# Inspector-Butters/light-client-consensus-specs

Measured on AMD Instinct MI355X. Metric: verified LightClientUpdates/sec (512-member committee), higher is better.
Workload: dtype u32 (381-bit Montgomery Fp on 12x32-bit limbs; SHA-256 words)

## Files before the change

### light-client-consensus-specs_amd/csrc/lcv_curve.hpp

```cpp
#pragma once
#include "lcv_tower.hpp"

namespace lcv {

LCV_FN void f_add(fp& r, const fp& a, const fp& b) { fp_add(r, a, b); }
LCV_FN void f_add(fp2& r, const fp2& a, const fp2& b) { fp2_add(r, a, b); }
LCV_FN void f_sub(fp& r, const fp& a, const fp& b) { fp_sub(r, a, b); }
LCV_FN void f_sub(fp2& r, const fp2& a, const fp2& b) { fp2_sub(r, a, b); }
LCV_FN void f_dbl(fp& r, const fp& a) { fp_dbl(r, a); }
LCV_FN void f_dbl(fp2& r, const fp2& a) { fp2_dbl(r, a); }
LCV_FN void f_neg(fp& r, const fp& a) { fp_neg(r, a); }
LCV_FN void f_neg(fp2& r, const fp2& a) { fp2_neg(r, a); }
LCV_FN void f_mul(fp& r, const fp& a, const fp& b) { fp_mul(r, a, b); }
LCV_FN void f_mul(fp2& r, const fp2& a, const fp2& b) { fp2_mul(r, a, b); }
LCV_FN void f_sqr(fp& r, const fp& a) { fp_sqr(r, a); }
LCV_FN void f_sqr(fp2& r, const fp2& a) { fp2_sqr(r, a); }
LCV_FN void f_inv(fp& r, const fp& a) { fp_inv(r, a); }
LCV_FN void f_inv(fp2& r, const fp2& a) { fp2_inv(r, a); }
LCV_FN bool f_is_zero(const fp& a) { return fp_is_zero(a); }
LCV_FN bool f_is_zero(const fp2& a) { return fp2_is_zero(a); }
LCV_FN bool f_eq(const fp& a, const fp& b) { return fp_eq(a, b); }
LCV_FN bool f_eq(const fp2& a, const fp2& b) { return fp2_eq(a, b); }
LCV_FN void f_one(fp& r) { fp_one(r); }
LCV_FN void f_one(fp2& r) { fp2_one(r); }
// ... 195 lines not shown
  if (xz) return aflag ? PT_BAD : PT_INF;
  if (!fp_raw_lt_p(xr)) return PT_BAD;
  fp x, g, y, chk, four;
  fp_to_mont(x, xr);
  fp_sqr(g, x);
  fp_mul(g, g, x);
  LCV_FP_SET(four, LCV_FOUR_INIT);
  fp_add(g, g, four);
  fp_pow_p1d4(y, g);
  fp_sqr(chk, y);
  if (!fp_eq(chk, g)) return PT_BAD;
  if (fp_is_large(y) != (aflag != 0)) fp_neg(y, y);
  r.x = x;
  r.y = y;
  return PT_OK;
}

LCV_FN void g1_compress(uint8_t* out, const g1a& p, bool inf) {
  if (inf) {
    out[0] = 0xc0;
    for (int i = 1; i < 48; ++i) out[i] = 0;
    return;
  }
  fp_to_be48(out, p.x);
  out[0] |= 0x80 | (fp_is_large(p.y) ? 0x20 : 0);
}

LCV_FN bool g1_in_subgroup(const g1a& p) {
  g1j t, u;
  jac_from_aff(t, p);
  LCV_NOUNROLL for (int i = 62; i >= 0; --i) {
    jac_dbl(t, t);
    if ((LCV_X_ABS >> i) & 1ull) jac_madd(t, t, p);
  }
  u = t;
  LCV_NOUNROLL for (int i = 62; i >= 0; --i) {
    jac_dbl(u, u);
    if ((LCV_X_ABS >> i) & 1ull) jac_add(u, u, t);
  }
  if (jac_is_inf(u)) return false;
  fp z2, z3, beta, a, b, ny;
  fp_sqr(z2, u.z);
  fp_mul(z3, z2, u.z);
  LCV_FP_SET(beta, LCV_G1_BETA_INIT);
  fp_mul(a, beta, p.x);
  fp_mul(a, a, z2);
  fp_neg(ny, p.y);
  fp_mul(b, ny, z3);
  return fp_eq(a, u.x) && fp_eq(b, u.y);
}

LCV_FN void g2_generator(g2a& r) { LCV_FP2_SET(r.x, LCV_G2X); LCV_FP2_SET(r.y, LCV_G2Y); }

LCV_FN int g2_decompress(g2a& r, const uint8_t* in) {
  const uint32_t b0 = in[0];
  const uint32_t cflag = (b0 >> 7) & 1u, bflag = (b0 >> 6) & 1u, aflag = (b0 >> 5) & 1u;
  fp x1r, x0r;
  fp_raw_from_be48(x1r, in);
  x1r.v[11] &= 0x1fffffffu;
  fp_raw_from_be48(x0r, in + 48);
  const uint32_t xz = (fp_is_zero(x1r) && fp_is_zero(x0r)) ? 1u : 0u;
  if (!cflag || bflag != xz) return PT_BAD;
  if (xz) return aflag ? PT_BAD : PT_INF;
  if (!fp_raw_lt_p(x1r) || !fp_raw_lt_p(x0r)) return PT_BAD;
  fp2 x, g, y, b;
  fp_to_mont(x.c0, x0r);
  fp_to_mont(x.c1, x1r);
  fp2_sqr(g, x);
  fp2_mul(g, g, x);
  LCV_FP2_SET(b, LCV_B2);
  fp2_add(g, g, b);
  if (!fp2_sqrt(y, g)) return PT_BAD;
  const bool large = fp_is_zero(y.c1) ? fp_is_large(y.c0) : fp_is_large(y.c1);
  if (large != (aflag != 0)) fp2_neg(y, y);
  r.x = x;
  r.y = y;
  return PT_OK;
}

LCV_FN void g2_compress(uint8_t* out, const g2a& p, bool inf) {
  if (inf) {
    out[0] = 0xc0;
    for (int i = 1; i < 96; ++i) out[i] = 0;
    return;
  }
  fp_to_be48(out, p.x.c1);
  fp_to_be48(out + 48, p.x.c0);
  const bool large = fp_is_zero(p.y.c1) ? fp_is_large(p.y.c0) : fp_is_large(p.y.c1);
  out[0] |= 0x80 | (large ? 0x20 : 0);
}

LCV_FN void g2_psi(g2j& r, const g2j& p) {
  fp2 cx, cy;
  LCV_FP2_SET(cx, LCV_PSI_CX);
  LCV_FP2_SET(cy, LCV_PSI_CY);
  fp2_conj(r.x, p.x);
  fp2_mul(r.x, r.x, cx);
  fp2_conj(r.y, p.y);
  fp2_mul(r.y, r.y, cy);
  fp2_conj(r.z, p.z);
}

LCV_FN bool g2_in_subgroup(const g2a& p) {
  g2j t;
  jac_mul_xabs_aff(t, p);
  if (jac_is_inf(t)) return false;
  fp2 cx, cy, px, py, z2, z3, a, b;
  LCV_FP2_SET(cx, LCV_PSI_CX);
  LCV_FP2_SET(cy, LCV_PSI_CY);
  fp2_conj(px, p.x);
  fp2_mul(px, px, cx);
  fp2_conj(py, p.y);
  fp2_mul(py, py, cy);
  fp2_sqr(z2, t.z);
  fp2_mul(z3, z2, t.z);
  fp2_mul(a, px, z2);
  fp2_mul(b, py, z3);
  fp2_neg(b, b);
  return fp2_eq(a, t.x) && fp2_eq(b, t.y);
}

LCV_FN void g2_clear_cofactor(g2j& r, const g2j& p) {
  g2j t1, t2, t3, u;
  jac_mul_x(t1, p);
  g2_psi(t2, p);
  jac_dbl(t3, p);
  g2_psi(t3, t3);
  g2_psi(t3, t3);
  jac_neg(u, t2);
  jac_add(t3, t3, u);
  jac_add(t2, t1, t2);
// ... 10 lines not shown
```

### light-client-consensus-specs_amd/csrc/lcv_field.hpp

```cpp
#pragma once
#include "lcv_common.hpp"
#include "lcv_consts.inc"
#include "lcv_col28.hpp"
#include "lcv_wave.hpp"

namespace lcv {

struct fp { uint32_t v[12]; };
struct fp2 { fp c0, c1; };

#define LCV_FP_SET(r, INIT) do { constexpr uint32_t _lcv_k[12] = INIT; LCV_UNROLL for (int _i = 0; _i < 12; ++_i) (r).v[_i] = _lcv_k[_i]; } while (0)
#define LCV_FP2_SET(r, NAME) do { LCV_FP_SET((r).c0, NAME##_C0); LCV_FP_SET((r).c1, NAME##_C1); } while (0)

LCV_FN void fp_zero(fp& r) { LCV_UNROLL for (int i = 0; i < 12; ++i) r.v[i] = 0; }
LCV_FN void fp_one(fp& r) { LCV_FP_SET(r, LCV_ONE_INIT); }
LCV_FN bool fp_is_zero(const fp& a) {
  uint32_t x = 0;
  LCV_UNROLL for (int i = 0; i < 12; ++i) x |= a.v[i];
  return x == 0;
}
LCV_FN bool fp_eq(const fp& a, const fp& b) {
  uint32_t x = 0;
  LCV_UNROLL for (int i = 0; i < 12; ++i) x |= a.v[i] ^ b.v[i];
  return x == 0;
// ... 172 lines not shown
#else
LCV_FN void fp_sqr(fp& r, const fp& a) { fp_mul(r, a, a); }
#endif

#define LCV_DEF_POW(fname, EXPARR, NBITS)                                  \
  LCV_FN void fname(fp& r, const fp& a) {                                  \
    fp acc = a;                                                            \
    LCV_NOUNROLL for (int i = (NBITS) - 2; i >= 0; --i) {                  \
      fp_sqr(acc, acc);                                                    \
      if ((EXPARR[i >> 5] >> (i & 31)) & 1u) fp_mul(acc, acc, a);          \
    }                                                                      \
    r = acc;                                                               \
  }
LCV_DEF_POW(fp_inv_fermat, LCV_EXP_P_MINUS_2, LCV_EXP_P_MINUS_2_BITS)
#define LCV_DEF_POW_W4(fname, EXPARR, NBITS)                                              \
  LCV_FN void fname(fp& r, const fp& a) {                                                 \
    fp tab[8], a2;                                                                        \
    tab[0] = a;                                                                           \
    fp_sqr(a2, a);                                                                        \
    LCV_UNROLL for (int k = 1; k < 8; ++k) fp_mul(tab[k], tab[k - 1], a2);               \
    fp acc = a;                                                                           \
    bool started = false;                                                                 \
    int i = (NBITS) - 1;                                                                  \
    LCV_NOUNROLL while (i >= 0) {                                                         \
      if (!((EXPARR[i >> 5] >> (i & 31)) & 1u)) {                                         \
        fp_sqr(acc, acc);                                                                 \
        --i;                                                                              \
        continue;                                                                         \
      }                                                                                   \
      int j = i - 3 < 0 ? 0 : i - 3;                                                      \
      while (!((EXPARR[j >> 5] >> (j & 31)) & 1u)) ++j;                                   \
      uint32_t w = 0;                                                                     \
      for (int k = i; k >= j; --k) {                                                      \
        w = (w << 1) | ((EXPARR[k >> 5] >> (k & 31)) & 1u);                               \
        if (started) fp_sqr(acc, acc);                                                    \
      }                                                                                   \
      fp m = tab[0];                                                                      \
      LCV_UNROLL for (int k = 1; k < 8; ++k) if ((w >> 1) == (uint32_t)k) m = tab[k];     \
      if (started) fp_mul(acc, acc, m); else acc = m;                                     \
      started = true;                                                                     \
      i = j - 1;                                                                          \
    }                                                                                     \
    r = acc;                                                                              \
  }
#ifndef LCV_POW_LF
#if defined(LCV_CPU_FAST)
#define LCV_POW_LF 0
#elif defined(LCV_HOSTSIM)
#define LCV_POW_LF 1
#else
#define LCV_POW_LF 2
#endif
#endif
#if LCV_POW_LF
LCV_FN void fp_lf_in(uint32_t L[14], const fp& a) {
  fp c, t;
  LCV_FP_SET(c, LCV_2E392_RAW_INIT);
  fp_mul(t, a, c);
  sop_to28<12, 14>(L, t.v);
}
LCV_FN void fp_lf_out(fp& r, const uint32_t L[14]) {
  uint32_t w[12];
  LCV_UNROLL for (int k = 0; k < 12; ++k) {
    const int b = 32 * k, j = b / 28, s = b % 28;
    uint32_t x = L[j] >> s;
    if (j + 1 < 14) x |= L[j + 1] << (28 - s);
    if (s > 24 && j + 2 < 14) x |= L[j + 2] << (56 - s);
    w[k] = x;
  }
  fp t, c;
  fp_reduce_once(t.v, w);
  LCV_FP_SET(c, LCV_2E376_RAW_INIT);
  fp_mul(r, t, c);
}
#define LCV_POW_WB (LCV_POW_LF == 2 ? 3 : 4)
#define LCV_POW_TAB(k, q) tabh[k][q]
#define LCV_POW_TAB_DECL uint32_t tabh[1 << (LCV_POW_WB - 1)][14];
#define LCV_POW_TAB_GET(m, idx)                                                           \
  LCV_UNROLL for (int q = 0; q < 14; ++q) m[q] = tabh[0][q];                              \
  LCV_UNROLL for (int k = 1; k < (1 << (LCV_POW_WB - 1)); ++k)                             \
    if ((idx) == (uint32_t)k) LCV_UNROLL for (int q = 0; q < 14; ++q) m[q] = tabh[k][q];
#define LCV_DEF_POW_LF(fname, EXPARR, NBITS)                                              \
  LCV_FN void fname(fp& r, const fp& a_) {                                                \
    uint32_t a[14], t[14], a2[14], acc[14];                                               \
    LCV_POW_TAB_DECL                                                                      \
    fp_lf_in(a, a_);                                                                      \
    LCV_UNROLL for (int j = 0; j < 14; ++j) LCV_POW_TAB(0, j) = a[j];                     \
    fp_sqr_lf(a2, a);                                                                     \
    LCV_UNROLL for (int j = 0; j < 14; ++j) t[j] = a[j];                                  \
    LCV_UNROLL for (int k = 1; k < (1 << (LCV_POW_WB - 1)); ++k) {                         \
      fp_mul_lf(t, t, a2);                                                                \
      LCV_UNROLL for (int j = 0; j < 14; ++j) LCV_POW_TAB(k, j) = t[j];                   \
    }                                                                                     \
    LCV_UNROLL for (int j = 0; j < 14; ++j) acc[j] = a[j];                                \
    bool started = false;                                                                 \
    int i = (NBITS) - 1;                                                                  \
    LCV_NOUNROLL while (i >= 0) {                                                         \
      if (!((EXPARR[i >> 5] >> (i & 31)) & 1u)) {                                         \
        fp_sqr_lf(acc, acc);                                                              \
        --i;                                                                              \
        continue;                                                                         \
      }                                                                                   \
      int j = i - (LCV_POW_WB - 1) < 0 ? 0 : i - (LCV_POW_WB - 1);                         \
      while (!((EXPARR[j >> 5] >> (j & 31)) & 1u)) ++j;                                   \
      uint32_t w = 0;                                                                     \
      for (int k = i; k >= j; --k) {                                                      \
        w = (w << 1) | ((EXPARR[k >> 5] >> (k & 31)) & 1u);                               \
        if (started) fp_sqr_lf(acc, acc);                                                 \
      }                                                                                   \
      uint32_t m[14];                                                                     \
      LCV_POW_TAB_GET(m, w >> 1)                                                          \
      if (started) fp_mul_lf(acc, acc, m);                                                \
      else LCV_UNROLL for (int q = 0; q < 14; ++q) acc[q] = m[q];                         \
      started = true;                                                                     \
      i = j - 1;                                                                          \
    }                                                                                     \
    fp_lf_out(r, acc);                                                                    \
  }
#if defined(__HIP_DEVICE_COMPILE__) && LCV_POW_LF == 3
#define LCV_DEF_POW_WAVE(fname, SCHED, NSCHED)                                            \
  LCV_FN void fname(fp& r, const fp& a_) {                                                \
    WaveTabs T;                                                                           \
    wv_tabs(T);                                                                           \
    uint32_t L[14];                                                                       \
    fp_lf_in(L, a_);                                                                      \
    const uint32_t a = wv_scatter(L);                                                     \
    uint32_t tab[8];                                                                      \
    tab[0] = a;                                                                           \
    const uint32_t a2 = wv_mul(a, a, T);                                                  \
    LCV_UNROLL for (int k = 1; k < 8; ++k) tab[k] = wv_mul(tab[k - 1], a2, T);            \
    uint32_t e = SCHED[0], acc = tab[0];                                                  \
    LCV_UNROLL for (int k = 1; k < 8; ++k) acc = (e >> 16) == (uint32_t)k ? tab[k] : acc; \
    LCV_NOUNROLL for (int t = 1; t < (NSCHED); ++t) {                                     \
      e = SCHED[t];                                                                       \
      LCV_NOUNROLL for (uint32_t q = e & 0xFFFFu; q > 0; --q) acc = wv_mul(acc, acc, T);  \
      const uint32_t idx = e >> 16;                                                       \
      if (idx != 0xFFFFu) {                                                               \
        uint32_t m = tab[0];                                                              \
        LCV_UNROLL for (int k = 1; k < 8; ++k) m = idx == (uint32_t)k ? tab[k] : m;        \
        acc = wv_mul(acc, m, T);                                                          \
      }                                                                                   \
    }                                                                                     \
    wv_gather(L, acc);                                                                    \
    fp_lf_out(r, L);                                                                      \
  }
// ... 157 lines not shown
    eta = by_divsteps30(eta, (uint32_t)f.v[0], (uint32_t)g.v[0], t);
    by_update_de(d, e, t);
    by_update_fg(f, g, t);
    int32_t z = 0;
    LCV_UNROLL for (int k = 0; k < 13; ++k) z |= g.v[k];
    if (z == 0) break;
  }
  uint32_t x[13];
  LCV_UNROLL for (int w = 0; w < 13; ++w) x[w] = 0;
  LCV_UNROLL for (int k = 0; k < 12; ++k) {
    const int b = 30 * k, w = b >> 5, s = b & 31;
    x[w] |= (uint32_t)d.v[k] << s;
    if (s > 2) x[w + 1] |= (uint32_t)d.v[k] >> (32 - s);
  }
  x[11] |= (uint32_t)d.v[12] << 8;
  x[12] = (uint32_t)(d.v[12] >> 24);
  LCV_UNROLL for (int pass = 0; pass < 2; ++pass) {
    const uint32_t m = 0u - (x[12] >> 31);
    uint32_t c = 0;
    LCV_UNROLL for (int j = 0; j < 12; ++j) x[j] = addc32(x[j], PL[j] & m, c, c);
    x[12] = x[12] + c;
  }
  uint32_t nz = 0;
  LCV_UNROLL for (int j = 0; j < 12; ++j) nz |= x[j];
  const uint32_t neg = (f.v[12] < 0 && nz != 0) ? 0xFFFFFFFFu : 0u;
  fp y;
  uint32_t br = 0;
  LCV_UNROLL for (int j = 0; j < 12; ++j) {
    const uint32_t n = subc32(PL[j], x[j], br, br);
    y.v[j] = neg ? n : x[j];
  }
  fp r3;
  LCV_FP_SET(r3, LCV_R3_INIT);
  fp_mul(r, y, r3);
}

LCV_FN void fp_inv(fp& r, const fp& a) { fp_inv_by(r, a); }

LCV_FN void fp2_zero(fp2& r) { fp_zero(r.c0); fp_zero(r.c1); }
LCV_FN void fp2_one(fp2& r) { fp_one(r.c0); fp_zero(r.c1); }
LCV_FN bool fp2_is_zero(const fp2& a) { return fp_is_zero(a.c0) && fp_is_zero(a.c1); }
LCV_FN bool fp2_eq(const fp2& a, const fp2& b) { return fp_eq(a.c0, b.c0) && fp_eq(a.c1, b.c1); }
LCV_FN void fp2_sel(fp2& r, bool c, const fp2& a, const fp2& b) { fp_sel(r.c0, c, a.c0, b.c0); fp_sel(r.c1, c, a.c1, b.c1); }
LCV_FN void fp2_add(fp2& r, const fp2& a, const fp2& b) { fp_add(r.c0, a.c0, b.c0); fp_add(r.c1, a.c1, b.c1); }
LCV_FN void fp2_sub(fp2& r, const fp2& a, const fp2& b) { fp_sub(r.c0, a.c0, b.c0); fp_sub(r.c1, a.c1, b.c1); }
LCV_FN void fp2_dbl(fp2& r, const fp2& a) { fp_dbl(r.c0, a.c0); fp_dbl(r.c1, a.c1); }
LCV_FN void fp2_neg(fp2& r, const fp2& a) { fp_neg(r.c0, a.c0); fp_neg(r.c1, a.c1); }
LCV_FN void fp2_half(fp2& r, const fp2& a) { fp_half(r.c0, a.c0); fp_half(r.c1, a.c1); }
LCV_FN void fp2_conj(fp2& r, const fp2& a) { r.c0 = a.c0; fp_neg(r.c1, a.c1); }
LCV_FN void fp2_mul_fp(fp2& r, const fp2& a, const fp& s) { fp_mul(r.c0, a.c0, s); fp_mul(r.c1, a.c1, s); }

LCV_FN void fp2_mul(fp2& r, const fp2& a, const fp2& b) {
  fp t0, t1, t2, t3;
  fp_mul(t0, a.c0, b.c0);
  fp_mul(t1, a.c1, b.c1);
  fp_add(t2, a.c0, a.c1);
  fp_add(t3, b.c0, b.c1);
  fp_mul(t2, t2, t3);
  fp_sub(r.c0, t0, t1);
  fp_sub(t2, t2, t0);
  fp_sub(r.c1, t2, t1);
}
LCV_FN void fp2_sqr(fp2& r, const fp2& a) {
  fp t0, t1, t2;
  fp_add(t0, a.c0, a.c1);
  fp_sub(t1, a.c0, a.c1);
  fp_mul(t2, a.c0, a.c1);
  fp_mul(r.c0, t0, t1);
  fp_dbl(r.c1, t2);
}
LCV_FN void fp2_mul_xi(fp2& r, const fp2& a) {
  fp t;
  fp_sub(t, a.c0, a.c1);
  fp_add(r.c1, a.c0, a.c1);
  r.c0 = t;
}
LCV_FN void fp2_inv(fp2& r, const fp2& a) {
  fp t0, t1;
  fp_sqr(t0, a.c0);
  fp_sqr(t1, a.c1);
  fp_add(t0, t0, t1);
  fp_inv(t1, t0);
  fp_mul(r.c0, a.c0, t1);
  fp_mul(t0, a.c1, t1);
  fp_neg(r.c1, t0);
}
LCV_FN void fp2_norm(fp& n, const fp2& a) {
  fp t;
  fp_sqr(n, a.c0);
  fp_sqr(t, a.c1);
  fp_add(n, n, t);
}

LCV_FN bool fp2_sqrt_alpha(fp2& y, const fp2& a, const fp& alpha) {
  const bool a1z = fp_is_zero(a.c1);
  fp delta;
  fp_add(delta, a.c0, alpha);
  fp_half(delta, delta);
  fp_sel(delta, a1z, a.c0, delta);
  fp t, c, s;
  fp_pow_p3d4(t, delta);
  fp_mul(c, t, delta);
  fp_mul(s, c, t);
  fp one;
  fp_one(one);
  const bool s_one = fp_eq(s, one);
  fp u, nu;
  fp_half(u, a.c1);
  fp_mul(u, u, t);
  fp_neg(nu, u);
  fp zero;
  fp_zero(zero);
  const bool first = a1z ? (s_one || fp_is_zero(delta)) : s_one;
  fp y0a, y1a;
  fp_sel(y0a, a1z, zero, nu);
  fp_sel(y1a, a1z, zero, u);
  fp_sel(y.c0, first, c, y0a);
  fp_sel(y.c1, first, y1a, c);
  fp2 chk;
  fp2_sqr(chk, y);
  return fp2_eq(chk, a);
}
LCV_FN bool fp2_sqrt(fp2& y, const fp2& a) {
  fp n, alpha;
  fp2_norm(n, a);
  fp_pow_p1d4(alpha, n);
  return fp2_sqrt_alpha(y, a, alpha);
}
LCV_FN bool fp2_is_square_alpha(const fp2& a, fp& alpha) {
  fp n, chk;
  fp2_norm(n, a);
  fp_pow_p1d4(alpha, n);
  fp_sqr(chk, alpha);
  return fp_eq(chk, n);
}
LCV_FN uint32_t fp2_sgn0(const fp2& a) {
  fp r0, r1;
  fp_from_mont(r0, a.c0);
  fp_from_mont(r1, a.c1);
  const uint32_t sign0 = r0.v[0] & 1u;
  const uint32_t zero0 = fp_is_zero(r0) ? 1u : 0u;
  const uint32_t sign1 = r1.v[0] & 1u;
  return sign0 | (zero0 & sign1);
}

}
```

### light-client-consensus-specs_amd/csrc/lcv_functors.hpp

```cpp
#pragma once
#include "lcv_items.hpp"

using namespace lcv;

struct F_nsc_team {
  BatchDev B; CommitteeDev C; Work W;
  static constexpr uint32_t TEAM = NSC_TEAM, LDS_WORDS = NSC_LDS, SHARED_WORDS = 0;
  LCV_HD uint32_t rounds() const { return NSC_ROUNDS; }
  LCV_HD void operator()(uint32_t j, uint32_t lane, uint32_t r, uint32_t* lds, uint32_t*) const { item_nsc_team(j, lane, r, lds, B, C, W); }
};
struct F_pre { BatchDev B; CommitteeDev C; Params P; Work W; LCV_HD void operator()(uint32_t i) const { item_pre(i, B, C, P, W); } };
struct F_sigroot { BatchDev B; Params P; Work W; LCV_HD void operator()(uint32_t i) const { item_sigroot(i, B, P, W); } };
struct F_h2c_map { Work W; LCV_HD void operator()(uint32_t t) const { item_h2c_map(t, W); } };
struct F_sig { BatchDev B; Work W; LCV_HD void operator()(uint32_t i) const { item_sig(i, B, W); } };
struct F_h2c_map_lat { Work W; LCV_HD void operator()(uint32_t t) const { item_h2c_map(t, W); } };
struct F_sig_lat { BatchDev B; Work W; LCV_HD void operator()(uint32_t i) const { item_sig(i, B, W); } };
struct F_agg { BatchDev B; CommitteeDev C; Work W; LCV_HD void operator()(uint32_t i) const { item_agg(i, B, C, W); } };
struct F_agg_fold { Work W; uint32_t m; LCV_HD void operator()(uint32_t) const { item_agg_fold(m, W); } };
struct F_verdict { Work W; LCV_HD void operator()(uint32_t i) const { item_verdict(i, W); } };
struct F_key { CommitteeDev C; LCV_HD void operator()(uint32_t t) const { item_committee_key(t, C); } };
struct F_agg_team {
  BatchDev B; CommitteeDev C; Work W;
  static constexpr uint32_t TEAM = AGG_TEAM, LDS_WORDS = AGG_LDS, SHARED_WORDS = 0;
  LCV_HD uint32_t rounds() const { return AGG_ROUNDS; }
  LCV_HD void operator()(uint32_t i, uint32_t lane, uint32_t r, uint32_t* lds, uint32_t*) const {
    item_agg_team(i, lane, r, lds, B, C, W);
  }
};
struct F_sum {
  CommitteeDev C;
  static constexpr uint32_t TEAM = SUM_TEAM, LDS_WORDS = SUM_LDS, SHARED_WORDS = 0;
  LCV_HD uint32_t rounds() const { return SUM_ROUNDS; }
  LCV_HD void operator()(uint32_t c, uint32_t lane, uint32_t r, uint32_t* lds, uint32_t*) const {
    item_committee_sum_team(c, lane, r, lds, C);
  }
};

struct F_msg_import {
  const uint8_t* msg; Work W;
  LCV_HD void operator()(uint32_t i) const {
    h256 m;
    LCV_UNROLL for (int k = 0; k < 8; ++k) m.w[k] = ld_be32(msg + 32 * (size_t)i + 4 * k);
    soa_st_h256(W.msg, W.cap, i, m);
  }
};
struct F_msg_import_b0 {
  const uint8_t* msg; uint64_t len; Work W;
  LCV_HD void operator()(uint32_t i) const {
    h256 b0;
    xmd_b0_bytes(b0, msg, len);
    soa_st_h256(W.msg, W.cap, i, b0);
  }
};
struct F_merkle {
  const uint8_t* leaf; const uint8_t* branch; const uint8_t* root; uint8_t* out; uint32_t depth; uint64_t index;
  LCV_HD void operator()(uint32_t i) const {
    h256 l, r;
    ld_chunk(l, leaf + 32 * (size_t)i);
    ld_chunk(r, root + 32 * (size_t)i);
    out[i] = merkle_branch_ok(l, branch + (size_t)32 * depth * i, (int)depth, index, r) ? 1 : 0;
  }
};
struct F_htr_sc {
  const uint8_t* sc; uint8_t* out;
  LCV_HD void operator()(uint32_t i) const {
    h256 r;
    htr_sync_committee(r, sc + (size_t)K_SC * i);
// ... 137 lines not shown
```

### light-client-consensus-specs_amd/csrc/lcv_h2c.hpp

```cpp
#pragma once
#include "lcv_curve.hpp"
#include "lcv_sha.hpp"

namespace lcv {

LCV_FN void xmd_next(h256& out, const h256& b0, const h256& prev, uint32_t i) {
  constexpr uint32_t C1T[8] = LCV_XMD_C1_TAIL_INIT;
  constexpr uint32_t C2[16] = LCV_XMD_C2_INIT;
  uint32_t st[8], blk[16];
  sha256_iv(st);
  LCV_UNROLL for (int k = 0; k < 8; ++k) { blk[k] = b0.w[k] ^ prev.w[k]; blk[8 + k] = C1T[k]; }
  blk[8] |= i << 24;
  sha256_compress(st, blk);
  LCV_UNROLL for (int k = 0; k < 16; ++k) blk[k] = C2[k];
  sha256_compress(st, blk);
  LCV_UNROLL for (int k = 0; k < 8; ++k) out.w[k] = st[k];
}

LCV_FN void xmd_b0(h256& b0, const h256& msg) {
  constexpr uint32_t H1[8] = LCV_XMD_H1_INIT;
  constexpr uint32_t B2T[8] = LCV_XMD_B2_TAIL_INIT;
  constexpr uint32_t B3[16] = LCV_XMD_B3_INIT;
  uint32_t st[8], blk[16];
  LCV_UNROLL for (int k = 0; k < 8; ++k) { st[k] = H1[k]; blk[k] = msg.w[k]; blk[8 + k] = B2T[k]; }
  sha256_compress(st, blk);
  LCV_UNROLL for (int k = 0; k < 16; ++k) blk[k] = B3[k];
  sha256_compress(st, blk);
  LCV_UNROLL for (int k = 0; k < 8; ++k) b0.w[k] = st[k];
}

LCV_FN void fp_from_xmd64(fp& r, const h256& hi, const h256& lo) {
  fp h, l, c, t;
  LCV_UNROLL for (int k = 0; k < 8; ++k) { h.v[k] = hi.w[7 - k]; l.v[k] = lo.w[7 - k]; }
  LCV_UNROLL for (int k = 8; k < 12; ++k) { h.v[k] = 0; l.v[k] = 0; }
  LCV_FP_SET(c, LCV_C256_INIT);
  fp_mul(t, h, c);
  LCV_FP_SET(c, LCV_R2_INIT);
  fp_mul(r, l, c);
  fp_add(r, r, t);
}

LCV_FN void iso_map_g2(g2j& r, const fp2& x, const fp2& y) {
  fp2 x2, x3, xn, xd, yn, yd, t, c;
  fp2_sqr(x2, x);
  fp2_mul(x3, x2, x);
  LCV_FP2_SET(c, LCV_ISO_XNUM3); fp2_mul(xn, c, x3);
  LCV_FP2_SET(c, LCV_ISO_XNUM2); fp2_mul(t, c, x2); fp2_add(xn, xn, t);
  LCV_FP2_SET(c, LCV_ISO_XNUM1); fp2_mul(t, c, x); fp2_add(xn, xn, t);
  LCV_FP2_SET(c, LCV_ISO_XNUM0); fp2_add(xn, xn, c);
  LCV_FP2_SET(c, LCV_ISO_XDEN1); fp2_mul(t, c, x); fp2_add(xd, x2, t);
  LCV_FP2_SET(c, LCV_ISO_XDEN0); fp2_add(xd, xd, c);
  LCV_FP2_SET(c, LCV_ISO_YNUM3); fp2_mul(yn, c, x3);
  LCV_FP2_SET(c, LCV_ISO_YNUM2); fp2_mul(t, c, x2); fp2_add(yn, yn, t);
  LCV_FP2_SET(c, LCV_ISO_YNUM1); fp2_mul(t, c, x); fp2_add(yn, yn, t);
  LCV_FP2_SET(c, LCV_ISO_YNUM0); fp2_add(yn, yn, c);
  LCV_FP2_SET(c, LCV_ISO_YDEN2); fp2_mul(t, c, x2); fp2_add(yd, x3, t);
  LCV_FP2_SET(c, LCV_ISO_YDEN1); fp2_mul(t, c, x); fp2_add(yd, yd, t);
  LCV_FP2_SET(c, LCV_ISO_YDEN0); fp2_add(yd, yd, c);
  fp2 yd2, xd3;
  fp2_sqr(yd2, yd);
  fp2_mul(r.z, xd, yd);
  fp2_mul(r.x, xn, xd);
  fp2_mul(r.x, r.x, yd2);
  fp2_sqr(xd3, xd);
  fp2_mul(xd3, xd3, xd);
  fp2_mul(t, xd3, yd2);
  fp2_mul(t, t, yn);
  fp2_mul(r.y, t, y);
}

LCV_FN void sswu_e2prime(fp2& xo, fp2& yo, const fp2& u) {
  fp2 A, B, Z, t, u2, zu2, den, x1, gx1, x2, gx2, x, gx, y, one, c;
  LCV_FP2_SET(A, LCV_ISO_A);
  LCV_FP2_SET(B, LCV_ISO_B);
  LCV_FP2_SET(Z, LCV_SSWU_Z);
  fp2_one(one);
  fp2_sqr(u2, u);
  fp2_mul(zu2, Z, u2);
  fp2_sqr(den, zu2);
  fp2_add(den, den, zu2);
  const bool den0 = fp2_is_zero(den);
  fp2_inv(t, den);
  fp2_add(t, t, one);
  LCV_FP2_SET(c, LCV_SSWU_NEGB_OVER_A);
  fp2_mul(x1, c, t);
  LCV_FP2_SET(c, LCV_SSWU_B_OVER_ZA);
  fp2_sel(x1, den0, c, x1);
  fp2_sqr(t, x1);
  fp2_mul(gx1, t, x1);
  fp2_mul(t, A, x1);
  fp2_add(gx1, gx1, t);
  fp2_add(gx1, gx1, B);
  fp2_mul(x2, zu2, x1);
  fp2_sqr(t, x2);
  fp2_mul(gx2, t, x2);
  fp2_mul(t, A, x2);
  fp2_add(gx2, gx2, t);
  fp2_add(gx2, gx2, B);
  fp alpha;
  const bool sq1 = fp2_is_square_alpha(gx1, alpha);
  fp2_sel(x, sq1, x1, x2);
  fp2_sel(gx, sq1, gx1, gx2);
  fp nu, alpha2, c2;
  fp2_norm(nu, u);
  fp_sqr(alpha2, nu);
  fp_mul(alpha2, alpha2, nu);
  LCV_FP_SET(c2, LCV_SSWU_ALPHA2_C_INIT);
  fp_mul(alpha2, alpha2, c2);
  fp_mul(alpha2, alpha2, alpha);
  fp alpha_sel;
  fp_sel(alpha_sel, sq1, alpha, alpha2);
  fp2_sqrt_alpha(y, gx, alpha_sel);
  if (fp2_sgn0(u) != fp2_sgn0(y)) fp2_neg(y, y);
  xo = x;
  yo = y;
}


LCV_FN void map_to_curve_g2(g2j& r, const fp2& u) {
  fp2 x, y;
  sswu_e2prime(x, y, u);
  iso_map_g2(r, x, y);
}

LCV_FN void xmd_b0_bytes(h256& b0, const uint8_t* msg, uint64_t len) {
  constexpr uint32_t H1[8] = LCV_XMD_H1_INIT;
  const char* dst = "BLS_SIG_BLS12381G2_XMD:SHA-256_SSWU_RO_POP_";
  uint32_t st[8], blk[16];
  LCV_UNROLL for (int k = 0; k < 8; ++k) st[k] = H1[k];
  const uint64_t body = len + 47;
  const uint64_t total = (body + 9 + 63) / 64 * 64;
  const uint64_t bits = (64 + body) * 8;
  LCV_NOUNROLL for (uint64_t base = 0; base < total; base += 64) {
    LCV_NOUNROLL for (int w = 0; w < 16; ++w) {
      uint32_t word = 0;
      for (int b = 0; b < 4; ++b) {
        const uint64_t k = base + 4 * w + b;
        uint32_t byte;
        if (k < len) byte = msg[k];
        else if (k == len) byte = 0x01;
        else if (k < len + 3) byte = 0x00;
        else if (k < len + 46) byte = (uint8_t)dst[k - len - 3];
        else if (k == len + 46) byte = 43;
        else if (k == body) byte = 0x80;
        else if (k >= total - 8) byte = (uint32_t)(bits >> (8 * (total - 1 - k))) & 0xFFu;
        else byte = 0;
        word = (word << 8) | byte;
      }
      blk[w] = word;
    }
    sha256_compress(st, blk);
  }
  LCV_UNROLL for (int k = 0; k < 8; ++k) b0.w[k] = st[k];
}

LCV_FN void hash_to_field_u_b0(fp2& u, const h256& b0, uint32_t m) {
  h256 prev, hi, lo;
  h256_zero(prev);
  LCV_NOUNROLL for (uint32_t k = 0; k <= m; ++k) {
    xmd_next(hi, b0, prev, 4 * k + 1);
    xmd_next(lo, b0, hi, 4 * k + 2);
    fp_from_xmd64(u.c0, hi, lo);
    xmd_next(hi, b0, lo, 4 * k + 3);
    xmd_next(lo, b0, hi, 4 * k + 4);
    fp_from_xmd64(u.c1, hi, lo);
// ... 43 lines not shown
```

### light-client-consensus-specs_amd/csrc/lcv_items.hpp

```cpp
#pragma once
#include "lcv_h2c.hpp"
#include "lcv_pairing.hpp"
#include "lcv_ssz.hpp"

namespace lcv {

struct BatchDev {
  const uint8_t* att_beacon;
  const uint8_t* att_exec;
  const uint8_t* att_branch;
  const uint8_t* fin_beacon;
  const uint8_t* fin_exec;
  const uint8_t* fin_branch;
  const uint8_t* nsc_pool;
  const uint32_t* nsc_index;
  const uint8_t* nsc_branch;
  const uint8_t* finality_branch;
  const uint8_t* bits;
  const uint8_t* sig;
  const uint64_t* sig_slot;
  uint32_t n;
  uint32_t npool;
};

// ... 186 lines not shown
  const bool fin_default = bytes_all_zero(fb, K_BEACON / 4) && bytes_all_zero(fe, K_EXEC / 4) &&
                           bytes_all_zero(fbr, K_EXEC_BRANCH / 4);
  if (!is_fin) {
    if (!fin_default) LCV_FAIL(7);
  } else {
    h256 leaf;
    if (fin_slot == 0) {
      if (!fin_default) LCV_FAIL(8);
      h256_zero(leaf);
    } else {
      if (!lc_header_valid(fb, fe, fbr, P.cfg)) LCV_FAIL(9);
      htr_beacon(leaf, fb);
    }
    if (!merkle_branch_ok(leaf, finb, 6, 41, state_root)) LCV_FAIL(10);
  }
  const uint32_t nflags = W.nsc_flags[pool];
  if (!is_sc) {
    if (!(nflags & 1u)) LCV_FAIL(11);
  } else {
    if (att_period == store_period && next_known && !(nflags & 2u)) LCV_FAIL(12);
    h256 leaf;
    soa_ld_h256(leaf, W.nsc_root, W.pool_cap, pool);
    if (!merkle_branch_ok(leaf, nbr, 5, 23, state_root)) LCV_FAIL(13);
  }
#undef LCV_FAIL
  W.comm_id[i] = sig_period != store_period ? 1u : 0u;
  W.pre_reason[i] = (uint8_t)reason;
}

LCV_FN void item_sigroot(uint32_t i, const BatchDev& B, const Params& P, const Work& W) {
  const uint8_t* ab = B.att_beacon + (size_t)K_BEACON * i;
  h256 gvr, msg;
  LCV_UNROLL for (int k = 0; k < 8; ++k) gvr.w[k] = P.gvr[k];
  signing_root(msg, ab, B.sig_slot[i], gvr, P.cfg);
  soa_st_h256(W.msg, W.cap, i, msg);
}

LCV_FN void st_g2a(uint32_t* base, size_t cap, size_t i, const g2a& q) {
  soa_st_fp2(base, cap, i, 0, q.x);
  soa_st_fp2(base, cap, i, 1, q.y);
}
LCV_FN void ld_g2a(g2a& q, const uint32_t* base, size_t cap, size_t i) {
  soa_ld_fp2(q.x, base, cap, i, 0);
  soa_ld_fp2(q.y, base, cap, i, 1);
}

LCV_FN void item_h2c_map(uint32_t t, const Work& W) {
  const uint32_t i = t >> 1, m = t & 1u;
  h256 msg;
  soa_ld_h256(msg, W.msg, W.cap, i);
  fp2 u, x, y;
  if (W.msg_b0) hash_to_field_u_b0(u, msg, m);
  else hash_to_field_u(u, msg, m);
  sswu_e2prime(x, y, u);
  soa_st_fp2(W.qmap, W.cap, i, 2 * m, x);
  soa_st_fp2(W.qmap, W.cap, i, 2 * m + 1, y);
}

LCV_FN void item_sig(uint32_t i, const BatchDev& B, const Work& W) {
  g2a s;
  fp2_zero(s.x);
  fp2_zero(s.y);
  const int st = g2_decompress(s, B.sig + 96 * (size_t)i);
  st_g2a(W.qs, W.cap, i, s);
  W.sig_status[i] = (uint8_t)st;
}

LCV_FN void ld_g1a_tbl(g1a& p, const uint32_t* pts, size_t idx) {
  const uint32_t* q = pts + idx * 24;
  LCV_UNROLL for (int k = 0; k < 12; ++k) { p.x.v[k] = q[k]; p.y.v[k] = q[12 + k]; }
}

LCV_FN void item_agg(uint32_t i, const BatchDev& B, const CommitteeDev& C, const Work& W) {
  const uint32_t c = W.comm_id[i];
  const uint32_t* bw = (const uint32_t*)(B.bits + 64 * (size_t)i);
  const uint32_t* bad = C.badmask + 16 * c;
  uint32_t pc = 0, anybad = 0;
  LCV_UNROLL for (int w = 0; w < 16; ++w) {
    pc += (uint32_t)__builtin_popcount(bw[w]);
    anybad |= bw[w] & bad[w];
  }
  const bool comp = pc > 256;
  g1j acc;
  if (comp) {
    const uint32_t* s = C.sum_all + 36 * c;
    LCV_UNROLL for (int k = 0; k < 12; ++k) { acc.x.v[k] = s[k]; acc.y.v[k] = s[12 + k]; acc.z.v[k] = s[24 + k]; }
  } else {
    jac_set_inf(acc);
  }
  const uint32_t* pts = C.pts + (size_t)c * 512 * 24;
  LCV_NOUNROLL for (int w = 0; w < 16; ++w) {
    uint32_t m = comp ? (~bw[w] & ~bad[w]) : bw[w];
    while (m) {
      const int b = __builtin_ctz(m);
      m &= m - 1;
      g1a p;
      ld_g1a_tbl(p, pts, 32 * w + b);
      if (comp) fp_neg(p.y, p.y);
      jac_madd(acc, acc, p);
    }
  }
  const bool inf = jac_is_inf(acc);
  g1a a;
  jac_to_aff(a, acc);
  soa_st_fp(W.pk, W.cap, i, 0, a.x);
  soa_st_fp(W.pk, W.cap, i, 1, a.y);
  W.agg_status[i] = (uint8_t)(anybad ? PT_BAD : (inf || pc == 0 ? PT_INF : PT_OK));
}

LCV_FN void ld_g1j_lds(g1j& p, const uint32_t* s) {
  LCV_UNROLL for (int k = 0; k < 12; ++k) { p.x.v[k] = s[k]; p.y.v[k] = s[12 + k]; p.z.v[k] = s[24 + k]; }
}
LCV_FN void st_g1j_lds(uint32_t* s, const g1j& p) {
  LCV_UNROLL for (int k = 0; k < 12; ++k) { s[k] = p.x.v[k]; s[12 + k] = p.y.v[k]; s[24 + k] = p.z.v[k]; }
}

// ... 148 lines not shown
```

### light-client-consensus-specs_amd/csrc/lcv_k_h2c.hip

```cpp
#define LCV_KERNEL_UNIT 1
#define LCV_HD __device__
#include "lcv_launch.hpp"
#include "lcv_functors.hpp"

LCV_INSTANTIATE(F_h2c_map)
```

### light-client-consensus-specs_amd/csrc/lcv_k_sig.hip

```cpp
#define LCV_KERNEL_UNIT 1
#define LCV_HD __device__
#include "lcv_launch.hpp"
#include "lcv_functors.hpp"

LCV_INSTANTIATE(F_sig)
```

### light-client-consensus-specs_amd/csrc/lcv_launch.hpp

```cpp
#pragma once
#include <hip/hip_runtime.h>
#include <stdint.h>

template <class F> hipError_t lcv_hip_launch(const F& f, uint32_t n, hipStream_t s);
template <class F> hipError_t lcv_hip_launch_team(const F& f, uint32_t n, hipStream_t s);
template <class F> hipError_t lcv_hip_launch_sop(const F& f, uint32_t n, hipStream_t s, uint32_t g = 0);
template <class F> hipError_t lcv_hip_launch_sop_fan(const F& f, uint32_t n, hipStream_t s);

#ifdef LCV_KERNEL_UNIT
template <class F>
__global__ __launch_bounds__(64, 1) void k_items(F f, uint32_t n) {
  const uint32_t i = blockIdx.x * 64u + threadIdx.x;
  if (i < n) f(i);
}
template <class F>
__global__ __launch_bounds__(64, 1) void k_wave(F f, uint32_t n) {
  (void)n;
  f(blockIdx.x);
}
template <class F> hipError_t lcv_hip_launch(const F& f, uint32_t n, hipStream_t s) {
#if defined(LCV_WAVE_ITEMS)
  hipLaunchKernelGGL(k_wave<F>, dim3(n), dim3(64), 0, s, f, n);
#else
  const uint32_t blocks = (n + 63u) / 64u;
  hipLaunchKernelGGL(k_items<F>, dim3(blocks), dim3(64), 0, s, f, n);
#endif
  return hipGetLastError();
}
template <class F>
__global__ __launch_bounds__(64) __attribute__((amdgpu_num_vgpr(168))) void k_team(F f, uint32_t n) {
  constexpr uint32_t T = F::TEAM, G = 64 / F::TEAM;
  __shared__ uint32_t lds[F::SHARED_WORDS + G * F::LDS_WORDS];
  const uint32_t team = threadIdx.x / T, lane = threadIdx.x % T;
  const uint32_t item = blockIdx.x * G + team;
  const bool active = team < G && item < n;
  uint32_t* my = lds + F::SHARED_WORDS + (team < G ? team : 0) * F::LDS_WORDS;
  const uint32_t R = f.rounds();
  for (uint32_t r = 0; r < R; ++r) {
    if (active) f(item, lane, r, my, lds);
    __syncthreads();
  }
}
template <class F> hipError_t lcv_hip_launch_team(const F& f, uint32_t n, hipStream_t s) {
  constexpr uint32_t G = 64 / F::TEAM;
  const uint32_t blocks = (n + G - 1) / G;
  hipLaunchKernelGGL(k_team<F>, dim3(blocks), dim3(64), 0, s, f, n);
  return hipGetLastError();
}
#define LCV_SOP_QP_WORDS 128u
template <class F> __global__ void k_sop(F f, uint32_t n, uint32_t g);
template <class F> hipError_t lcv_hip_launch_sop(const F& f, uint32_t n, hipStream_t s, uint32_t g) {
  constexpr uint32_t G = 64 / F::TEAM;
  if (g == 0 || g > G) g = G;
  const uint32_t blocks = (n + g - 1) / g;
  const size_t lds_bytes = 4 * (size_t)(F::SHARED_WORDS + LCV_SOP_QP_WORDS + g * F::LDS_WORDS);
  hipLaunchKernelGGL(k_sop<F>, dim3(blocks), dim3(64), lds_bytes, s, f, n, g);
  return hipGetLastError();
}
constexpr uint32_t LCV_FAN_ROW_MAX_TEAM = 16;
template <class F> constexpr bool lcv_fan_rows() { return F::TEAM <= LCV_FAN_ROW_MAX_TEAM; }
template <class F> constexpr uint32_t lcv_fan_threads() {
  constexpr uint32_t a = ((F::TEAM * F::MAXK * F::FAN_PARTS + 63) / 64) * 64;
  constexpr uint32_t b = lcv_fan_rows<F>() ? ((16 * F::TEAM + 63) / 64) * 64 : 0;
  return a > b ? a : b;
// ... 15 lines not shown
```

Before: 1.782 million.

## Cut register pressure in h2c map and sig decompress to allow 3 waves/EU

Restructures the SSWU map and G2 signature decompression so live values are parked in global scratch and recomputed, instead of being held across the long exponentiation chains. The pow window table moves from registers to per-lane LDS. These kernels get amdgpu_waves_per_eu(3) and a raised wave priority, aiming for higher occupancy to hide latency. The cost is extra global and LDS traffic plus recomputation of cheap values such as x1 and g(x). Spilling becomes a risk if the register budget is still exceeded.

```diff
diff --git a/light-client-consensus-specs_amd/csrc/lcv_curve.hpp b/light-client-consensus-specs_amd/csrc/lcv_curve.hpp
--- a/light-client-consensus-specs_amd/csrc/lcv_curve.hpp
+++ b/light-client-consensus-specs_amd/csrc/lcv_curve.hpp
@@ -271,31 +271,77 @@
 
 LCV_FN void g2_generator(g2a& r) { LCV_FP2_SET(r.x, LCV_G2X); LCV_FP2_SET(r.y, LCV_G2Y); }
 
-LCV_FN int g2_decompress(g2a& r, const uint8_t* in) {
-  const uint32_t b0 = in[0];
-  const uint32_t cflag = (b0 >> 7) & 1u, bflag = (b0 >> 6) & 1u, aflag = (b0 >> 5) & 1u;
-  fp x1r, x0r;
+LCV_FN void g2_raw_x(fp& x1r, fp& x0r, const uint8_t* in) {
   fp_raw_from_be48(x1r, in);
   x1r.v[11] &= 0x1fffffffu;
   fp_raw_from_be48(x0r, in + 48);
-  const uint32_t xz = (fp_is_zero(x1r) && fp_is_zero(x0r)) ? 1u : 0u;
-  if (!cflag || bflag != xz) return PT_BAD;
-  if (xz) return aflag ? PT_BAD : PT_INF;
-  if (!fp_raw_lt_p(x1r) || !fp_raw_lt_p(x0r)) return PT_BAD;
-  fp2 x, g, y, b;
+}
+LCV_FN void g2_x_gx(fp2& x, fp2& g, const fp& x1r, const fp& x0r) {
+  fp2 b;
   fp_to_mont(x.c0, x0r);
   fp_to_mont(x.c1, x1r);
   fp2_sqr(g, x);
   fp2_mul(g, g, x);
   LCV_FP2_SET(b, LCV_B2);
   fp2_add(g, g, b);
-  if (!fp2_sqrt(y, g)) return PT_BAD;
+}
+LCV_FN int g2_decode_head(uint32_t& aflag, const uint8_t* in) {
+  const uint32_t b0 = in[0];
+  const uint32_t cflag = (b0 >> 7) & 1u, bflag = (b0 >> 6) & 1u;
+  aflag = (b0 >> 5) & 1u;
+  fp x1r, x0r;
+  g2_raw_x(x1r, x0r, in);
+  const uint32_t xz = (fp_is_zero(x1r) && fp_is_zero(x0r)) ? 1u : 0u;
+  if (!cflag || bflag != xz) return PT_BAD;
+  if (xz) return aflag ? PT_BAD : PT_INF;
+  if (!fp_raw_lt_p(x1r) || !fp_raw_lt_p(x0r)) return PT_BAD;
+  return PT_OK;
+}
+LCV_FN void g2_y_sign(fp2& y, uint32_t aflag) {
   const bool large = fp_is_zero(y.c1) ? fp_is_large(y.c0) : fp_is_large(y.c1);
   if (large != (aflag != 0)) fp2_neg(y, y);
+}
+LCV_FN int g2_decompress(g2a& r, const uint8_t* in) {
+  uint32_t aflag;
+  const int st = g2_decode_head(aflag, in);
+  if (st != PT_OK) return st;
+  fp x1r, x0r;
+  fp2 x, g, y;
+  g2_raw_x(x1r, x0r, in);
+  g2_x_gx(x, g, x1r, x0r);
+  if (!fp2_sqrt(y, g)) return PT_BAD;
+  g2_y_sign(y, aflag);
   r.x = x;
   r.y = y;
   return PT_OK;
 }
+#if LCV_CHAIN_SLOT
+template <class Park>
+LCV_FN int g2_decompress_slot(g2a& r, const uint8_t* in, const Park& park) {
+  uint32_t aflag;
+  const int st = g2_decode_head(aflag, in);
+  if (st != PT_OK) return st;
+  fp x1r, x0r, n, alpha;
+  fp2 x, g, y, chk;
+  g2_raw_x(x1r, x0r, in);
+  g2_x_gx(x, g, x1r, x0r);
+  park.st(g);
+  fp2_norm(n, g);
+  fp_pow_p1d4(alpha, n);
+  park.ld(g);
+  fp2_sqrt_alpha_nochk(y, g, alpha);
+  fp2_sqr(chk, y);
+  park.ld(g);
+  if (!fp2_eq(chk, g)) return PT_BAD;
+  g2_y_sign(y, aflag);
+  LCV_CHAIN_CUT_AT(in);
+  g2_raw_x(x1r, x0r, in);
+  fp_to_mont(r.x.c0, x0r);
+  fp_to_mont(r.x.c1, x1r);
+  r.y = y;
+  return PT_OK;
+}
+#endif
 
 LCV_FN void g2_compress(uint8_t* out, const g2a& p, bool inf) {
   if (inf) {
diff --git a/light-client-consensus-specs_amd/csrc/lcv_field.hpp b/light-client-consensus-specs_amd/csrc/lcv_field.hpp
--- a/light-client-consensus-specs_amd/csrc/lcv_field.hpp
+++ b/light-client-consensus-specs_amd/csrc/lcv_field.hpp
@@ -248,6 +248,15 @@
 #define LCV_POW_LF 2
 #endif
 #endif
+#if LCV_POW_LF == 2 && defined(__HIP_DEVICE_COMPILE__)
+#define LCV_CHAIN_SLOT 1
+#define LCV_CHAIN_CUT() asm volatile("" ::: "memory")
+#define LCV_CHAIN_CUT_AT(v) asm volatile("" : "+v"(v) : : "memory")
+#else
+#define LCV_CHAIN_SLOT 0
+#define LCV_CHAIN_CUT() ((void)0)
+#define LCV_CHAIN_CUT_AT(v) ((void)0)
+#endif
 #if LCV_POW_LF
 LCV_FN void fp_lf_in(uint32_t L[14], const fp& a) {
   fp c, t;
@@ -270,23 +279,36 @@
   fp_mul(r, t, c);
 }
 #define LCV_POW_WB (LCV_POW_LF == 2 ? 3 : 4)
-#define LCV_POW_TAB(k, q) tabh[k][q]
+#if LCV_CHAIN_SLOT
+LCV_FN uint32_t* fp_pow_tab_lds() {
+  __shared__ uint32_t tab[((1 << (LCV_POW_WB - 1)) - 1) * 14 * 64];
+  return tab + (threadIdx.x & 63u);
+}
+#define LCV_POW_TAB_DECL uint32_t* const tabl = fp_pow_tab_lds();
+#define LCV_POW_TAB_PUT(k, src)                                                           \
+  if ((k) > 0) LCV_UNROLL for (int q = 0; q < 14; ++q) tabl[(((k) - 1) * 14 + q) * 64] = src[q];
+#define LCV_POW_TAB_GET(m, idx)                                                           \
+  if ((idx) == 0u) { LCV_UNROLL for (int q = 0; q < 14; ++q) m[q] = a[q]; }               \
+  else { LCV_UNROLL for (int q = 0; q < 14; ++q) m[q] = tabl[(((idx) - 1u) * 14u + q) * 64u]; }
+#else
 #define LCV_POW_TAB_DECL uint32_t tabh[1 << (LCV_POW_WB - 1)][14];
+#define LCV_POW_TAB_PUT(k, src) LCV_UNROLL for (int q = 0; q < 14; ++q) tabh[k][q] = src[q];
 #define LCV_POW_TAB_GET(m, idx)                                                           \
   LCV_UNROLL for (int q = 0; q < 14; ++q) m[q] = tabh[0][q];                              \
   LCV_UNROLL for (int k = 1; k < (1 << (LCV_POW_WB - 1)); ++k)                             \
     if ((idx) == (uint32_t)k) LCV_UNROLL for (int q = 0; q < 14; ++q) m[q] = tabh[k][q];
+#endif
 #define LCV_DEF_POW_LF(fname, EXPARR, NBITS)                                              \
   LCV_FN void fname(fp& r, const fp& a_) {                                                \
     uint32_t a[14], t[14], a2[14], acc[14];                                               \
     LCV_POW_TAB_DECL                                                                      \
     fp_lf_in(a, a_);                                                                      \
-    LCV_UNROLL for (int j = 0; j < 14; ++j) LCV_POW_TAB(0, j) = a[j];                     \
+    LCV_POW_TAB_PUT(0, a)                                                                 \
     fp_sqr_lf(a2, a);                                                                     \
     LCV_UNROLL for (int j = 0; j < 14; ++j) t[j] = a[j];                                  \
     LCV_UNROLL for (int k = 1; k < (1 << (LCV_POW_WB - 1)); ++k) {                         \
       fp_mul_lf(t, t, a2);                                                                \
-      LCV_UNROLL for (int j = 0; j < 14; ++j) LCV_POW_TAB(k, j) = t[j];                   \
+      LCV_POW_TAB_PUT(k, t)                                                               \
     }                                                                                     \
     LCV_UNROLL for (int j = 0; j < 14; ++j) acc[j] = a[j];                                \
     bool started = false;                                                                 \
@@ -550,10 +572,10 @@
 
 LCV_FN void fp2_mul(fp2& r, const fp2& a, const fp2& b) {
   fp t0, t1, t2, t3;
+  fp_add(t2, a.c0, a.c1);
+  fp_add(t3, b.c0, b.c1);
   fp_mul(t0, a.c0, b.c0);
   fp_mul(t1, a.c1, b.c1);
-  fp_add(t2, a.c0, a.c1);
-  fp_add(t3, b.c0, b.c1);
   fp_mul(t2, t2, t3);
   fp_sub(r.c0, t0, t1);
   fp_sub(t2, t2, t0);
@@ -590,21 +612,21 @@
   fp_add(n, n, t);
 }
 
-LCV_FN bool fp2_sqrt_alpha(fp2& y, const fp2& a, const fp& alpha) {
-  const bool a1z = fp_is_zero(a.c1);
-  fp delta;
+LCV_FN void fp2_sqrt_delta(fp& delta, const fp2& a, const fp& alpha) {
   fp_add(delta, a.c0, alpha);
   fp_half(delta, delta);
-  fp_sel(delta, a1z, a.c0, delta);
-  fp t, c, s;
-  fp_pow_p3d4(t, delta);
+  fp_sel(delta, fp_is_zero(a.c1), a.c0, delta);
+}
+LCV_FN void fp2_sqrt_finish(fp2& y, const fp& a1, const fp& delta, const fp& t) {
+  const bool a1z = fp_is_zero(a1);
+  fp c, s;
   fp_mul(c, t, delta);
   fp_mul(s, c, t);
   fp one;
   fp_one(one);
   const bool s_one = fp_eq(s, one);
   fp u, nu;
-  fp_half(u, a.c1);
+  fp_half(u, a1);
   fp_mul(u, u, t);
   fp_neg(nu, u);
   fp zero;
@@ -615,6 +637,15 @@
   fp_sel(y1a, a1z, zero, u);
   fp_sel(y.c0, first, c, y0a);
   fp_sel(y.c1, first, y1a, c);
+}
+LCV_FN void fp2_sqrt_alpha_nochk(fp2& y, const fp2& a, const fp& alpha) {
+  fp delta, t;
+  fp2_sqrt_delta(delta, a, alpha);
+  fp_pow_p3d4(t, delta);
+  fp2_sqrt_finish(y, a.c1, delta, t);
+}
+LCV_FN bool fp2_sqrt_alpha(fp2& y, const fp2& a, const fp& alpha) {
+  fp2_sqrt_alpha_nochk(y, a, alpha);
   fp2 chk;
   fp2_sqr(chk, y);
   return fp2_eq(chk, a);
diff --git a/light-client-consensus-specs_amd/csrc/lcv_functors.hpp b/light-client-consensus-specs_amd/csrc/lcv_functors.hpp
--- a/light-client-consensus-specs_amd/csrc/lcv_functors.hpp
+++ b/light-client-consensus-specs_amd/csrc/lcv_functors.hpp
@@ -11,8 +11,8 @@
 };
 struct F_pre { BatchDev B; CommitteeDev C; Params P; Work W; LCV_HD void operator()(uint32_t i) const { item_pre(i, B, C, P, W); } };
 struct F_sigroot { BatchDev B; Params P; Work W; LCV_HD void operator()(uint32_t i) const { item_sigroot(i, B, P, W); } };
-struct F_h2c_map { Work W; LCV_HD void operator()(uint32_t t) const { item_h2c_map(t, W); } };
-struct F_sig { BatchDev B; Work W; LCV_HD void operator()(uint32_t i) const { item_sig(i, B, W); } };
+struct F_h2c_map { static constexpr uint32_t WAVES = 3; Work W; LCV_HD void operator()(uint32_t t) const { item_h2c_map(t, W); } };
+struct F_sig { static constexpr uint32_t WAVES = 3; BatchDev B; Work W; LCV_HD void operator()(uint32_t i) const { item_sig(i, B, W); } };
 struct F_h2c_map_lat { Work W; LCV_HD void operator()(uint32_t t) const { item_h2c_map(t, W); } };
 struct F_sig_lat { BatchDev B; Work W; LCV_HD void operator()(uint32_t i) const { item_sig(i, B, W); } };
 struct F_agg { BatchDev B; CommitteeDev C; Work W; LCV_HD void operator()(uint32_t i) const { item_agg(i, B, C, W); } };
diff --git a/light-client-consensus-specs_amd/csrc/lcv_h2c.hpp b/light-client-consensus-specs_amd/csrc/lcv_h2c.hpp
--- a/light-client-consensus-specs_amd/csrc/lcv_h2c.hpp
+++ b/light-client-consensus-specs_amd/csrc/lcv_h2c.hpp
@@ -69,14 +69,15 @@
   fp2_mul(r.y, t, y);
 }
 
-LCV_FN void sswu_e2prime(fp2& xo, fp2& yo, const fp2& u) {
-  fp2 A, B, Z, t, u2, zu2, den, x1, gx1, x2, gx2, x, gx, y, one, c;
-  LCV_FP2_SET(A, LCV_ISO_A);
-  LCV_FP2_SET(B, LCV_ISO_B);
+LCV_FN void sswu_zu2(fp2& zu2, const fp2& u) {
+  fp2 Z, u2;
   LCV_FP2_SET(Z, LCV_SSWU_Z);
-  fp2_one(one);
   fp2_sqr(u2, u);
   fp2_mul(zu2, Z, u2);
+}
+LCV_FN void sswu_x1(fp2& x1, const fp2& zu2) {
+  fp2 den, t, one, c;
+  fp2_one(one);
   fp2_sqr(den, zu2);
   fp2_add(den, den, zu2);
   const bool den0 = fp2_is_zero(den);
@@ -86,21 +87,23 @@
   fp2_mul(x1, c, t);
   LCV_FP2_SET(c, LCV_SSWU_B_OVER_ZA);
   fp2_sel(x1, den0, c, x1);
-  fp2_sqr(t, x1);
-  fp2_mul(gx1, t, x1);
-  fp2_mul(t, A, x1);
-  fp2_add(gx1, gx1, t);
-  fp2_add(gx1, gx1, B);
-  fp2_mul(x2, zu2, x1);
-  fp2_sqr(t, x2);
-  fp2_mul(gx2, t, x2);
-  fp2_mul(t, A, x2);
-  fp2_add(gx2, gx2, t);
-  fp2_add(gx2, gx2, B);
-  fp alpha;
-  const bool sq1 = fp2_is_square_alpha(gx1, alpha);
-  fp2_sel(x, sq1, x1, x2);
-  fp2_sel(gx, sq1, gx1, gx2);
+}
+LCV_FN void sswu_g(fp2& gx, const fp2& x) {
+  fp2 A, B, t;
+  LCV_FP2_SET(A, LCV_ISO_A);
+  LCV_FP2_SET(B, LCV_ISO_B);
+  fp2_sqr(t, x);
+  fp2_add(t, t, A);
+  fp2_mul(gx, t, x);
+  fp2_add(gx, gx, B);
+}
+LCV_FN bool sswu_is_sq(const fp2& gx1, const fp& alpha) {
+  fp n, chk;
+  fp2_norm(n, gx1);
+  fp_sqr(chk, alpha);
+  return fp_eq(chk, n);
+}
+LCV_FN void sswu_alpha_sel(fp& alpha_sel, bool sq1, const fp2& u, const fp& alpha) {
   fp nu, alpha2, c2;
   fp2_norm(nu, u);
   fp_sqr(alpha2, nu);
@@ -108,9 +111,22 @@
   LCV_FP_SET(c2, LCV_SSWU_ALPHA2_C_INIT);
   fp_mul(alpha2, alpha2, c2);
   fp_mul(alpha2, alpha2, alpha);
-  fp alpha_sel;
   fp_sel(alpha_sel, sq1, alpha, alpha2);
-  fp2_sqrt_alpha(y, gx, alpha_sel);
+}
+LCV_FN void sswu_e2prime(fp2& xo, fp2& yo, const fp2& u) {
+  fp2 zu2, x1, x2, g, x, y;
+  sswu_zu2(zu2, u);
+  sswu_x1(x1, zu2);
+  sswu_g(g, x1);
+  fp n, alpha, alpha_sel;
+  fp2_norm(n, g);
+  fp_pow_p1d4(alpha, n);
+  const bool sq1 = sswu_is_sq(g, alpha);
+  fp2_mul(x2, zu2, x1);
+  fp2_sel(x, sq1, x1, x2);
+  sswu_alpha_sel(alpha_sel, sq1, u, alpha);
+  sswu_g(g, x);
+  fp2_sqrt_alpha_nochk(y, g, alpha_sel);
   if (fp2_sgn0(u) != fp2_sgn0(y)) fp2_neg(y, y);
   xo = x;
   yo = y;
diff --git a/light-client-consensus-specs_amd/csrc/lcv_items.hpp b/light-client-consensus-specs_amd/csrc/lcv_items.hpp
--- a/light-client-consensus-specs_amd/csrc/lcv_items.hpp
+++ b/light-client-consensus-specs_amd/csrc/lcv_items.hpp
@@ -262,16 +262,76 @@
   fp2 u, x, y;
   if (W.msg_b0) hash_to_field_u_b0(u, msg, m);
   else hash_to_field_u(u, msg, m);
+#if LCV_CHAIN_SLOT
+  const auto park_st = [&](uint32_t slot, const fp2& a) {
+    uint32_t j = t;
+    LCV_CHAIN_CUT_AT(j);
+    soa_st_fp2(W.qmap, W.cap, j >> 1, 2 * (j & 1u) + slot, a);
+  };
+  const auto park_ld = [&](fp2& r, uint32_t slot) {
+    uint32_t j = t;
+    LCV_CHAIN_CUT_AT(j);
+    soa_ld_fp2(r, W.qmap, W.cap, j >> 1, 2 * (j & 1u) + slot);
+  };
+  fp2 zu2, x1, g;
+  fp n, alpha, alpha_sel;
+  park_st(1, u);
+  sswu_zu2(zu2, u);
+  sswu_x1(x1, zu2);
+  park_st(0, x1);
+  sswu_g(g, x1);
+  fp2_norm(n, g);
+  fp_pow_p1d4(alpha, n);
+  park_ld(x1, 0);
+  sswu_g(g, x1);
+  const bool sq1 = sswu_is_sq(g, alpha);
+  park_ld(u, 1);
+  sswu_zu2(zu2, u);
+  park_ld(x1, 0);
+  fp2_mul(x, zu2, x1);
+  park_ld(x1, 0);
+  fp2_sel(x, sq1, x1, x);
+  park_ld(u, 1);
+  sswu_alpha_sel(alpha_sel, sq1, u, alpha);
+  fp2 keep;
+  fp_zero(keep.c1);
+  keep.c1.v[0] = fp2_sgn0(u);
+  park_st(0, x);
+  sswu_g(g, x);
+  keep.c0 = g.c1;
+  park_st(1, keep);
+  fp delta, r;
+  fp2_sqrt_delta(delta, g, alpha_sel);
+  fp_pow_p3d4(r, delta);
+  park_ld(keep, 1);
+  fp2_sqrt_finish(y, keep.c0, delta, r);
+  if (keep.c1.v[0] != fp2_sgn0(y)) fp2_neg(y, y);
+  park_st(1, y);
+#else
   sswu_e2prime(x, y, u);
   soa_st_fp2(W.qmap, W.cap, i, 2 * m, x);
   soa_st_fp2(W.qmap, W.cap, i, 2 * m + 1, y);
+#endif
 }
 
 LCV_FN void item_sig(uint32_t i, const BatchDev& B, const Work& W) {
   g2a s;
+#if LCV_CHAIN_SLOT
+  struct {
+    const Work& W; uint32_t i;
+    LCV_FN void st(const fp2& a) const { uint32_t j = i; LCV_CHAIN_CUT_AT(j); soa_st_fp2(W.qs, W.cap, j, 0, a); }
+    LCV_FN void ld(fp2& a) const { uint32_t j = i; LCV_CHAIN_CUT_AT(j); soa_ld_fp2(a, W.qs, W.cap, j, 0); }
+  } park{W, i};
+  const int st = g2_decompress_slot(s, B.sig + 96 * (size_t)i, park);
+  if (st != PT_OK) {
+    fp2_zero(s.x);
+    fp2_zero(s.y);
+  }
+#else
   fp2_zero(s.x);
   fp2_zero(s.y);
   const int st = g2_decompress(s, B.sig + 96 * (size_t)i);
+#endif
   st_g2a(W.qs, W.cap, i, s);
   W.sig_status[i] = (uint8_t)st;
 }
diff --git a/light-client-consensus-specs_amd/csrc/lcv_k_h2c.hip b/light-client-consensus-specs_amd/csrc/lcv_k_h2c.hip
--- a/light-client-consensus-specs_amd/csrc/lcv_k_h2c.hip
+++ b/light-client-consensus-specs_amd/csrc/lcv_k_h2c.hip
@@ -1,5 +1,5 @@
 #define LCV_KERNEL_UNIT 1
-#define LCV_HD __device__
+#define LCV_HD __device__ __forceinline__
 #include "lcv_launch.hpp"
 #include "lcv_functors.hpp"
 
diff --git a/light-client-consensus-specs_amd/csrc/lcv_k_sig.hip b/light-client-consensus-specs_amd/csrc/lcv_k_sig.hip
--- a/light-client-consensus-specs_amd/csrc/lcv_k_sig.hip
+++ b/light-client-consensus-specs_amd/csrc/lcv_k_sig.hip
@@ -1,5 +1,5 @@
 #define LCV_KERNEL_UNIT 1
-#define LCV_HD __device__
+#define LCV_HD __device__ __forceinline__
 #include "lcv_launch.hpp"
 #include "lcv_functors.hpp"
 
diff --git a/light-client-consensus-specs_amd/csrc/lcv_launch.hpp b/light-client-consensus-specs_amd/csrc/lcv_launch.hpp
--- a/light-client-consensus-specs_amd/csrc/lcv_launch.hpp
+++ b/light-client-consensus-specs_amd/csrc/lcv_launch.hpp
@@ -8,8 +8,11 @@
 template <class F> hipError_t lcv_hip_launch_sop_fan(const F& f, uint32_t n, hipStream_t s);
 
 #ifdef LCV_KERNEL_UNIT
+template <class F, class = void> struct lcv_items_waves { static constexpr uint32_t value = 1; };
+template <class F> struct lcv_items_waves<F, decltype((void)F::WAVES)> { static constexpr uint32_t value = F::WAVES; };
 template <class F>
-__global__ __launch_bounds__(64, 1) void k_items(F f, uint32_t n) {
+__global__ __launch_bounds__(64) __attribute__((amdgpu_waves_per_eu(lcv_items_waves<F>::value))) void k_items(F f, uint32_t n) {
+  if constexpr (lcv_items_waves<F>::value > 1) __builtin_amdgcn_s_setprio(3);
   const uint32_t i = blockIdx.x * 64u + threadIdx.x;
   if (i < n) f(i);
 }
```

Measured after the change: 1.748 million. 0.981x the previous value.
